# nemochina2008/soundgen_beta

Measured on AMD Instinct MI355X. Metric: synthesized audio samples/sec (whole node) @44.1 kHz; RMS error vs R ref, higher is better.
Workload: dtype fp32 (fp64 phase)

## Files before the change

### include/soundgen_hip.h

```cpp
#ifndef SOUNDGEN_HIP_H
#define SOUNDGEN_HIP_H

#include <stdint.h>

#ifdef __cplusplus
extern "C" {
#endif

#define SG_ABI_VERSION 5

enum {
  SG_OK = 0,
  SG_E_ARG = -1,
  SG_E_DOMAIN = -2,
  SG_E_RANDOM = -3,
  SG_E_UNSUPPORTED = -4,
  SG_E_DEVICE = -5,
  SG_E_CAPACITY = -6,
  SG_E_NOMEM = -7
};

typedef struct sg_anchors {
  int32_t n;
  const double* time;
// ... 114 lines not shown
void sg_plan_destroy(sg_plan* plan);
int64_t sg_plan_n_calls(const sg_plan* plan);
int64_t sg_plan_total_samples(const sg_plan* plan);
int sg_plan_lengths(const sg_plan* plan, int64_t* out_len, int64_t* out_off);
int sg_plan_status(const sg_plan* plan, int32_t* out_status);
int64_t sg_plan_device_bytes(const sg_plan* plan);
int sg_plan_upload(sg_ctx* ctx, sg_plan* plan);
int sg_plan_release_host(sg_plan* plan);
int sg_execute(sg_ctx* ctx, sg_plan* plan, float* d_out, void* stream);
int sg_execute_plans(sg_ctx* ctx, sg_plan* const* plans, float* const* d_outs, int n, void* stream);
int sg_set_profiling(sg_ctx* ctx, int on);
int sg_profile_read(sg_ctx* ctx, double* sine_ms_avg, int64_t* n);
#define SG_PROF_SINE_BANK 0
#define SG_PROF_STFT_OLA 1
int sg_profile_read_kernel(sg_ctx* ctx, int kernel, double* ms_avg, int64_t* n);
int sg_synchronize(sg_ctx* ctx);
int sg_execute_to_host(sg_ctx* ctx, sg_plan* plan, double* out_host);
const char* sg_plan_call_message(const sg_plan* plan, int64_t i);
int sg_plan_kernel_stats(const sg_plan* plan, int64_t* harm_samples,
                         int64_t* harm_terms, int64_t* harm_amp_bytes,
                         int64_t* fft_frames);
int sg_plan_table_stats(const sg_plan* plan, int64_t* tables, int64_t* samples, int64_t* terms);
int sg_plan_stft_stats(const sg_plan* plan, int64_t* samples, int64_t* alg_bytes, double* flops);
int sg_plan_sine_tasks(const sg_plan* plan, int64_t* counts);
int sg_plan_precision(const sg_plan* plan, int32_t* call_fp64, int64_t* fp64_frames, int64_t* fp64_tasks);
int sg_plan_conditioning(const sg_plan* plan, double* rho);
int sg_plan_noise_conditioning(const sg_plan* plan, double* rho);
int sg_plan_call_work(const sg_plan* plan, double* rows, double* fft_flops);
typedef struct sg_mel_params {
  double samplingRate;
  double windowLength;
  double overlap;
  double step;
  double throwaway;
  double maxFreq;
  int32_t penalizeLengthDif;
  int32_t pad;
} sg_mel_params;
int sg_mel_spec(sg_ctx* ctx, const double* wave, int64_t len, const sg_mel_params* p, double* out, int64_t cap,
                int32_t* nb, int32_t* nc);
int sg_compare_sounds_batch(sg_ctx* ctx, const double* target_spec, int32_t nb, int32_t nc_target,
                            const float* d_wave, const int64_t* offsets, const int64_t* lengths, int64_t n,
                            const sg_mel_params* p, int32_t methods, double* out, double* summary);
int sg_dtw_symmetric2(const double* x, int64_t n, const double* y, int64_t m, double* out);
typedef struct sg_ssm_params {
  double samplingRate;
// ... 216 lines not shown
```

### soundgen_beta_amd/batch.py

```python
import ctypes as C

import numpy as np

from . import _abi, native, rargs


class Marshalled:

    def __init__(self, calls):
        self.holder = h = rargs.Holder()
        n = self.n = len(calls)
        N = max(n, 1)
        descs = (_abi.sg_call_desc * N)()
        args = (_abi.sg_soundgen_args * N)()
        self._structs = [args]
        aw = rargs.ArgsWriter(h, args, N)
        fast, rand = [], []
        for i, c in enumerate(calls):
            kind = c.get("kind", "soundgen")
            if kind != "harmonics" and c.get("rng") is None:
                aw.add(i, c.get("args", {}))
                fast.append(i)
                rand.append(h.random_addrs(c.get("normals"), c.get("uniforms")))
                continue
# ... 130 lines not shown
        descs = m.descs
        self._descs = descs
        self.ptr = C.c_void_p()
        L = native.lib()
        native.check(L.sg_plan_batch(ctx.ptr if ctx else None, descs, n, C.byref(self.ptr)), ctx.ptr if ctx else None)
        self.n = n
        self.lengths = np.zeros(n, dtype=np.int64)
        self.offsets = np.zeros(n, dtype=np.int64)
        i64p = C.POINTER(C.c_int64)
        L.sg_plan_lengths(self.ptr, self.lengths.ctypes.data_as(i64p), self.offsets.ctypes.data_as(i64p))
        self.status = np.zeros(n, dtype=np.int32)
        L.sg_plan_status(self.ptr, self.status.ctypes.data_as(C.POINTER(C.c_int32)))
        self.total = int(L.sg_plan_total_samples(self.ptr))
        self.uploaded = False

    def message(self, i):
        return native.lib().sg_plan_call_message(self.ptr, i).decode()

    def stats(self):
        v = [C.c_int64() for _ in range(4)]
        native.lib().sg_plan_kernel_stats(self.ptr, *[C.byref(x) for x in v])
        w = [C.c_int64(), C.c_int64(), C.c_double()]
        native.lib().sg_plan_stft_stats(self.ptr, *[C.byref(x) for x in w])
        return dict(harm_samples=v[0].value, harm_terms=v[1].value, harm_amp_bytes=v[2].value,
                    fft_frames=v[3].value, stft_samples=w[0].value, stft_bytes=w[1].value, stft_flops=w[2].value)

    def sine_tasks(self):
        v = (C.c_int64 * 5)()
        native.check(native.lib().sg_plan_sine_tasks(self.ptr, v))
        return tuple(int(x) for x in v)

    def table_stats(self):
        v = [C.c_int64() for _ in range(3)]
        native.check(native.lib().sg_plan_table_stats(self.ptr, *[C.byref(x) for x in v]))
        return tuple(x.value for x in v)

    def noise_conditioning(self):
        v = np.zeros(self.n, dtype=np.float64)
        native.check(native.lib().sg_plan_noise_conditioning(self.ptr, v.ctypes.data_as(C.POINTER(C.c_double))))
        return v

    def conditioning(self):
        v = np.zeros(self.n, dtype=np.float64)
        native.check(native.lib().sg_plan_conditioning(self.ptr, v.ctypes.data_as(C.POINTER(C.c_double))))
        return v

    def precision(self):
        v = np.zeros(self.n, dtype=np.int32)
# ... 171 lines not shown
```

### soundgen_beta_amd/csrc/sg_api.cpp

```cpp
#include <hip/hip_runtime.h>

#include <algorithm>
#include <cmath>
#include <atomic>
#include <chrono>
#include <cstring>
#include <exception>
#include <memory>
#include <thread>
#include <string>
#include <vector>

#include "sg_plan.h"
#include "sg_exec.h"
#include "sg_amp.h"
#include "sg_prof.h"
#include "sg_mel.h"
#include "sg_launch.h"

#include <cstdio>
#include <cstdlib>

struct sg_plan {
  sg::Batch B;
// ... 654 lines not shown
  *harm_samples = plan->B.harm_samples;
  *harm_terms = plan->B.harm_terms;
  *harm_amp_bytes = plan->B.harm_amp_bytes;
  *fft_frames = plan->B.fft_frames;
  return SG_OK;
}

int sg_plan_table_stats(const sg_plan* plan, int64_t* tables, int64_t* samples, int64_t* terms) {
  if (!plan || !tables || !samples || !terms) return SG_E_ARG;
  *tables = plan->D.uploaded ? (int64_t)plan->D.tabjobs_host.size() : 0;
  *samples = plan->D.uploaded ? plan->D.tab_samples : 0;
  *terms = plan->D.uploaded ? plan->D.tab_terms : 0;
  return SG_OK;
}

int sg_plan_stft_stats(const sg_plan* plan, int64_t* samples, int64_t* alg_bytes, double* flops) {
  if (!plan) return SG_E_ARG;
  *samples = plan->B.stft_samples;
  *alg_bytes = plan->B.stft_bytes;
  *flops = plan->B.stft_flops;
  return SG_OK;
}

int sg_plan_sine_tasks(const sg_plan* plan, int64_t* counts) {
  if (!plan || !counts) return SG_E_ARG;
  const sg::DevicePlan& D = plan->D;
  counts[0] = (int64_t)D.tlong_host.size();
  counts[1] = (int64_t)D.tshort_host.size();
  counts[2] = (int64_t)D.tall_host.size();
  counts[3] = (int64_t)D.tallp_host.size();
  counts[4] = (int64_t)D.thp_host.size();
  return SG_OK;
}

int64_t sg_plan_amp_count(const sg_plan* plan) { return plan && !plan->host_released ? plan->B.amp_total : 0; }

int sg_plan_debug_amps(const sg_plan* plan, float* out, int64_t n) {
  if (!plan || plan->host_released || !out || n < plan->B.amp_total) return SG_E_ARG;
  const sg::Batch& B = plan->B;
  std::vector<double> lg((size_t)B.amp_lg_rows + 1);
  for (size_t k = 0; k < lg.size(); ++k) lg[k] = std::log2((double)(k + 1));
  for (const SgAmpJob& J : B.ampjobs)
    for (int32_t r = 0; r < J.Rp; ++r)
      for (int32_t g = 0; g < J.G; ++g) {
        float a;
        if (r >= J.R) a = 0.f;
// ... 387 lines not shown
```

### soundgen_beta_amd/csrc/sg_dev.h

```cpp
#pragma once
#include <stdint.h>

struct SgSeg {
  double t0;
  double c0, c1, c2, c3, c4;
};

struct SgEpoch {
  int64_t w_off;
  int64_t amp_off;
  int64_t knot_off;
  int32_t seg_off;
  int32_t nseg;
  int32_t n;
  int32_t G;
  int32_t R;
  int32_t u0;
  double x1, xG;
  double xby;
  double invD;
  int32_t dj0, dj1;
  int64_t dk0;
  int32_t syl;
  int32_t pad;
// ... 141 lines not shown

constexpr int SG_FFT_WG = 0;
constexpr int SG_FFT_WAVE = 1;
constexpr int SG_FFT_DFT = 2;
constexpr int SG_FFT_ODD = 3;
constexpr int SG_WAVE_STATE = 24;
constexpr int SG_FFT_WAVES = 8;

#ifndef SG_NOISE_WAVES
#define SG_NOISE_WAVES 12
#endif
constexpr int SG_FFT_WAVES_NOISE = SG_NOISE_WAVES;
constexpr int sg_fft_waves(int phase) { return phase == 0 ? SG_FFT_WAVES_NOISE : SG_FFT_WAVES; }
constexpr int SG_PF_SRC = 20;
constexpr int SG_PF_PAIR = 10;

constexpr int SG_FRAME_FILTER = 0;
constexpr int SG_FRAME_NOISE = 1;
struct SgFrame {
  int64_t src;
  int64_t env;
  int64_t dst;
};
struct SgFrame64 {
  int64_t src;
  int64_t env;
  int64_t dst;
  int32_t wl;
  int32_t mode;
};
constexpr int SG_F64W_M_HOST = 1102;
constexpr int32_t SG_F64_FILTER = 0;
constexpr int32_t SG_F64_NOISE = 1;
struct SgFrameGroup {
  int32_t geom, mode;
  int32_t f0, nf;
};

struct SgOla {
  int64_t frames;
  int64_t out;
  int64_t first, len, xlen;
  double h;
  int32_t nframes, wl;
  float scale;
  int32_t tile0;
// ... 130 lines not shown
```

### soundgen_beta_amd/csrc/sg_fft.hip

```cpp
#include <hip/hip_runtime.h>

#include <type_traits>

#include "sg_dev.h"
#include "sg_devfn.h"
#include "sg_fft64_dev.h"
#include "sg_roots.h"

namespace {

typedef float v2 __attribute__((ext_vector_type(2)));
__device__ __forceinline__ v2 V(float2 a) { return v2{a.x, a.y}; }
__device__ __forceinline__ float2 F(v2 a) { return make_float2(a.x, a.y); }
__device__ __forceinline__ v2 pfma(v2 a, v2 b, v2 c) { return __builtin_elementwise_fma(a, b, c); }
__device__ __forceinline__ v2 splat(float c) { return v2{c, c}; }
__device__ __forceinline__ v2 vmul(v2 a, v2 w) {
  v2 t, r;
  __asm__("v_pk_mul_f32 %0, %1, %2 op_sel_hi:[0,1]" : "=v"(t) : "v"(a), "v"(w));
  __asm__("v_pk_fma_f32 %0, %1, %2, %3 op_sel:[1,1,0] op_sel_hi:[1,0,1] neg_lo:[0,1,0]"
          : "=v"(r) : "v"(a), "v"(w), "v"(t));
  return r;
}
__device__ __forceinline__ v2 vmulc(v2 a, v2 w) {
  v2 t, r;
// ... 885 lines not shown
  auto bstart = [&](int f) -> int { return hi > 0 ? f * hi : (int)floor((double)f * h); };
  const int first = (int)O.first, len = (int)O.len;
  const float scale = O.scale;
  float* out = fs + O.out;
  float m = -INFINITY;
  constexpr bool FUSED = CM == 1102 && R0 == 29 && R1 == 19 && R2 == 2;
  constexpr int CR = FUSED ? 9 : CP;
  float2 C[CR], C2[FUSED ? 9 : 1];
#pragma unroll
  for (int r = 0; r < CR; ++r) C[r] = make_float2(0.f, 0.f);
#pragma unroll
  for (int r = 0; r < (FUSED ? 9 : 1); ++r) C2[r] = make_float2(0.f, 0.f);
  FramePf P;
  constexpr int W = MODE == SG_FRAME_NOISE ? SG_FFT_WAVES_NOISE : SG_FFT_WAVES;
  const float4* A29 = reinterpret_cast<const float4*>(twS + M * (4 + W));
#ifdef SG_STFT_STAMPS
  uint64_t st_accv[10] = {0, 0, 0, 0, 0, 0, 0, 0, 0, 0};
  uint64_t st_lastv = __builtin_amdgcn_s_memtime();
  uint64_t* st_acc = st_accv;
  uint64_t* st_last = &st_lastv;
#endif
  int bf = bstart(S.f0);
  for (int k = 0; k < S.nf; ++k) {
    {
      int Mk = M;
      if (!CM) __asm__ __volatile__("" : "+s"(Mk));
      frame_prefetch<FUSED && MODE == SG_FRAME_FILTER>(P, frames[S.fdev + k], mode, Mk, fl, fs, lane);
    }
    frame_front<CM, R0, R1, R2>(A, P, mode, g, twS, twN, ham, A29, lane SG_ST_ARGS);
    SG_ST(4);
    const float2* han2 = reinterpret_cast<const float2*>(han);
    const bool lastf = k == S.nf - 1;
    const int bn = lastf ? S.pb : bstart(S.f0 + k + 1);
    const int D = bn - bf;
    const bool direct = FUSED && MODE == SG_FRAME_NOISE && bf >= S.pa && bf - first >= 0 && bn - first <= len && D <= 1102;
    if constexpr (FUSED) {
      fft_wc<true, CM, R0, R1, R2, MODE == SG_FRAME_FILTER || SG_NOISE_MFMA, false>(A, twS, A29, lane SG_ST_ARGS);
      float* __restrict__ o = out + (bf - first);
      const bool o2 = ((O.out + bf - first) & 1) == 0;
#pragma unroll
      for (int q = 0; q < 9; ++q) {
        const int j = 64 * q + lane;
        if (j >= 551) continue;
        const float2 a = A[j], c = A[j + 551];
        const float2 t = cmulc(c, twS[550 + j]);
        const float2 y0 = F(pfma(V(cadd(a, t)), V(han2[j]), V(C[q])));
        A[j + 551] = F(pfma(V(csub(a, t)), V(han2[j + 551]), V(C2[q])));
        if (direct && 2 * j < D) {
          const float v0 = y0.x * scale, v1 = y0.y * scale;
          if (2 * j + 1 < D) {
            if (o2) *reinterpret_cast<float2*>(o + 2 * j) = make_float2(v0, v1);
            else {
              o[2 * j] = v0;
              o[2 * j + 1] = v1;
            }
            m = fmaxf(m, fmaxf(v0, v1));
          } else {
            o[2 * j] = v0;
            m = fmaxf(m, v0);
// ... 866 lines not shown
```

### soundgen_beta_amd/csrc/sg_plan.h

```cpp
#pragma once
#include <cstdint>
#include <functional>
#include <memory>
#include <utility>
#include <vector>

#include "sg_dev.h"
#include "sg_rmath.h"
#include "soundgen_hip.h"

namespace sg {

template <class T>
struct NoInitAlloc : std::allocator<T> {
  template <class U>
  struct rebind { using other = NoInitAlloc<U>; };
  NoInitAlloc() = default;
  template <class U>
  NoInitAlloc(const NoInitAlloc<U>&) noexcept {}
  T* allocate(size_t n) {
    if (n * sizeof(T) < SG_BULK_HUGE) return std::allocator<T>::allocate(n);
    return static_cast<T*>(bulk_alloc(n * sizeof(T)));
  }
  void deallocate(T* p, size_t n) noexcept {
// ... 115 lines not shown
  struct UGather {
    const double* src;
    int64_t n, dst, ntot;
  };
  std::vector<UGather> ugath;
  int64_t fu_total = 0, fu_base = 0;
  std::vector<float> ustream;
  std::vector<SgUJob> ujobs;
  std::vector<double> elog2;
  std::vector<int64_t> call_len, call_off;
  std::vector<int32_t> call_status;
  std::vector<int32_t> call_fp64;
  std::vector<double> call_rho;
  double rho_cur = 0;
  std::vector<double> call_rho_noise;
  double rho_noise_cur = 0;
  std::vector<std::string> call_msg;
  int64_t total_out = 0;
  int64_t harm_samples = 0, harm_terms = 0, harm_amp_bytes = 0, fft_frames = 0;
  double fft_flops = 0;
  std::vector<double> call_rows, call_flops;
  int64_t stft_bytes = 0, stft_samples = 0;
  double stft_flops = 0;
};

struct HarmProbe {
  int64_t t;
  double f0;
  std::vector<double> amp;
};
int64_t plan_harmonics(Batch& B, const double* pitch, int64_t len, const sg_harm_params& P,
                       const sg_anchors& amplAnchors, Rng& R, int64_t out_off, bool dry_run, bool to_fs = false,
                       int64_t* fs_off = nullptr, std::vector<HarmProbe>* probes = nullptr);
int64_t syllable_to_fp64(Batch& B, int s);
int64_t fh_alloc(Batch& B, int64_t n);

bool smooth_contour(const sg_anchors& an, int64_t len, bool thisIsPitch, int method, bool has_floor,
                    double vfloor, bool has_ceil, double vceil, vec& out, double sr = 16000);
SgContour contour_desc(Batch& B, const sg_anchors& an, int64_t L, bool has_floor, double vfloor,
                       bool has_ceil, double vceil, bool db, double sr);

void tile_syllables(Batch& B, int first_syl);

int64_t plan_soundgen(Batch& B, const sg_soundgen_args& a, Rng& R, int64_t out_off, int first_syl);
void restore_soundgen_tail(Batch& B, int first_syl);
void finalize_plan(Batch& B);
void finalize_spec(Batch& B);

int geometry(Batch& B, int wl);
int64_t fs_alloc(Batch& B, int64_t n);
int64_t fl_push(Batch& B, const double* v, int64_t n);
int plan_filter(Batch& B, int64_t sound, int64_t L, int wl, double overlap, int64_t env, int64_t env_nc,
                int64_t* out_len, int64_t* out_fs, bool hp = false);
bool plan_noise(Batch& B, Rng& R, int64_t len, const sg_anchors& noiseAnchors, double rolloffNoise,
                double attackLen, int wl, double sr, double overlap, const double* filterNoise, int64_t fnc,
                SgNoiseItem* item, int64_t filt_env = 0);
bool noise_to_fp64(Batch& B, const std::vector<int>& olas);
int64_t plan_envelope(Batch& B, Rng& R, double nrd, int64_t nc, const sg_formants* F, double formantDep,
                      double rolloffLip, const sg_anchors& mouthAnchors, double mouthOpenThres, double openMouthBoost,
                      double vocalTract, double temperature, double formDrift, double formDisp,
                      double formantDepStoch, double smoothLinearFactor, double sr, double speedSound,
                      double slope = 0);
vec sigmoid_half(double sr, double freq, double shape, double spikiness);

vec get_rolloff(const vec& pitch, int64_t nH, const vec& rolloff, const vec& rolloffOct, double rolloffParab,
                double rolloffParabHarm, const vec& rolloffKHz, double baseline, double throwaway, double sr,
                int64_t& H, double rolloffParabCeiling = NAN);
vec get_random_walk(Rng& R, int64_t len, double rw_range, double rw_smoothing, int method, const vec& trend,
                    bool trend_lazy_rnorm, bool draws_only = false);
void clumper(vec& s, const vec& minLen);
double noise_threshold(int which, double nonlinBalance);

}

namespace sg {
int plan_batch_ex(sg_ctx* ctx, const sg_call_desc* calls, int64_t n_calls, bool independent_draws, sg_plan** out,
// ... 5 lines not shown
```

### soundgen_beta_amd/csrc/sg_plan_soundgen.cpp

```cpp
#include <algorithm>
#include <atomic>
#include <cmath>
#include <cstdlib>
#include <cstring>
#include <optional>

#include "sg_plan.h"

namespace sg {

namespace {

constexpr int kNPV = 33;
const char* const kPVNames[kNPV] = {
    "repeatBout", "nSyl", "sylLen", "pauseLen", "temperature", "maleFemale", "creakyBreathy", "nonlinBalance",
    "nonlinDep", "jitterDep", "jitterLen", "vibratoFreq", "vibratoDep", "shimmerDep", "attackLen", "rolloff",
    "rolloffOct", "rolloffParab", "rolloffParabHarm", "rolloffKHz", "rolloffLip", "formantDep", "formantDepStoch",
    "vocalTract", "subFreq", "subDep", "shortestEpoch", "amDep", "amFreq", "amShape", "samplingRate",
    "windowLength", "rolloffNoise"};
const double kPV[kNPV][3] = {
    {1, 1, 20}, {1, 1, 10}, {300, 20, 5000}, {200, 20, 1000}, {.025, 0, 1}, {0, -1, 1}, {0, -1, 1},
    {0, 0, 100}, {50, 0, 100}, {3, 0, 24}, {1, 1, 100}, {5, 3, 10}, {0, 0, 3}, {0, 0, 100},
    {50, 0, 200}, {-12, -60, 0}, {-12, -30, 10}, {0, -50, 50}, {3, 1, 20}, {-6, -20, 0},
    {6, 0, 20}, {1, 0, 5}, {30, 0, 60}, {15.5, 2, 100}, {100, 10, 1000}, {100, 0, 500},
// ... 627 lines not shown
        ci.off = 0;
        B.items.push_back(ci);
        B.mixes[0].push_back(c);
      }
      zero_mix(at, Ls - at);
    } else {
      sound_fs = hp ? fh_alloc(B, std::max<int64_t>(Ls, 1)) : fs_alloc(B, std::max<int64_t>(Ls, 1));
      SgMix pre{};
      pre.dst = sound_fs;
      pre.len = Ls;
      pre.to_fs = hp ? 2 : 1;
      pre.base_kind = SG_BASE_NONE;
      ncontent = emit(sound, pre.item0);
      pre.nitems = ncontent;
      pre.mult = mult;
      B.mixes[0].push_back(pre);
    }
    Layout post;
    if (ncontent == 0) {
      post.items.push_back(raw_item(sound_fs, Ls, 0));
      post.len = Ls;
    } else {
      int64_t filt_fs = 0, Lf = 0;
      const int ola = plan_filter(B, sound_fs, Ls, wl, A.overlap, filt_env, nInt, &Lf, &filt_fs, hp);
      SgNoiseItem fi = raw_item(filt_fs, Lf, 0);
      fi.ola = ola;
      fi.flags = SG_ITEM_FILTER_OLA;
      post.items.push_back(fi);
      post.len = Lf;
    }
    if (postNoise)
      for (size_t s = 0; s < noises.size(); ++s) post.add(noises[s], noiseIp[s]);
    SgMix fin{};
    fin.to_fs = 0;
    fin.base_kind = SG_BASE_NONE;
    fin.len = post.len;
    fin.nitems = emit(post, fin.item0);
    fin.mult.kind = 0;
    if (A.amDep > 0) {
      const vec half = sigmoid_half(sr, A.amFreq, A.amShape, 1);
      fin.am_tab = fl_push(B, half.data(), (int64_t)half.size());
      fin.am_lo = (int32_t)half.size();
      fin.am_dep = (float)A.amDep;
    }
    if (b > 0) {
      const int64_t np = (int64_t)(A.pauseLen * sr / 1000);
      SgMix z{};
// ... 71 lines not shown
```

### soundgen_beta_amd/csrc/sg_plan_spec.cpp

```cpp
#include <algorithm>
#include <atomic>
#include <cmath>
#include <complex>
#include <cstdio>
#include <cstdlib>
#include <cstring>
#include <map>
#include <memory>
#include <mutex>
#include <string>

#include "sg_plan.h"
#include "sg_prof.h"

#ifndef SG_SEG_SORT
#define SG_SEG_SORT 1
#endif
#ifndef SG_ENV_SORT
#define SG_ENV_SORT 1
#endif

namespace sg {

namespace {
// ... 269 lines not shown
}

static int push_ola(Batch& B, int phase, int64_t frames, int64_t nframes, int wl, const IstftGeom& ig, int64_t first,
                    int64_t len, int64_t out, bool fused, bool f64 = false) {
  if (fused && ig.xlen >= (int64_t)1 << 31) throw SgError(SG_E_UNSUPPORTED, "istft: output longer than 2^31 samples");
  SgOla o{};
  o.fidx = f64 ? -1 : (int32_t)((int64_t)B.frames[phase].size() - nframes);
  o.fused = fused ? 1 : 0;
  o.frames = frames;
  o.out = out;
  o.first = first;
  o.len = len;
  o.xlen = ig.xlen;
  o.h = ig.h;
  o.nframes = (int32_t)nframes;
  o.wl = wl;
  o.scale = ig.scale;
  o.hi = (ig.h == std::floor(ig.h) && ig.h >= 1 && ig.h < 2147483647.0) ? (int32_t)ig.h : 0;
  B.olas[phase].push_back(o);
  return (int)B.olas[phase].size() - 1;
}

int plan_filter(Batch& B, int64_t sound, int64_t L, int wl, double overlap, int64_t env, int64_t env_nc,
                int64_t* out_len, int64_t* out_fs, bool hp) {
  ProfScope ps(PF_FILTER);
  const int gi = geometry(B, wl);
  const int64_t nr = wl / 2;
  const double by = (double)wl - overlap * (double)wl / 100;
  const vec step = r_seq_by(1, (double)std::max<int64_t>(1, L - wl), by);
  const int64_t nc = (int64_t)step.size();
  if (env_nc != 1 && env_nc != nc) throw SgError(SG_E_ARG, "formant filter: envelope columns != frames");
  for (double x0 : step)
    if ((int64_t)x0 - 1 + wl > L) throw SgError(SG_E_DOMAIN, "stft: frame beyond the sound");
  const bool fused = !hp && fusable(B.geoms[gi], (double)wl * (100 - overlap) / 100);
  const int64_t fr = fused ? 0 : fs_alloc(B, nc * wl);
  if (hp) {
    for (int64_t c = 0; c < nc; ++c) {
      SgFrame64 f{};
      f.src = sound + (int64_t)step[c] - 1;
      const int64_t col = env_nc == 1 ? 0 : c * nr;
      f.env = env < 0 ? env - col : env + col;
      f.dst = fr + c * wl;
      f.wl = wl;
      B.frames64.push_back(f);
    }
    const IstftGeom ig = istft_geom(wl, nc, overlap);
    const int64_t out = fs_alloc(B, ig.xlen);
    B.fft_frames += nc;
    B.fft_flops += 2 * 5.0 * wl * std::log2((double)wl) * (double)nc;
    *out_len = ig.xlen;
    *out_fs = out;
    return push_ola(B, 1, fr, nc, wl, ig, 0, ig.xlen, out, false, true);
  }
  for (int64_t c = 0; c < nc; ++c) {
    SgFrame f{};
    f.src = sound + (int64_t)step[c] - 1;
    const int64_t col = env_nc == 1 ? 0 : c * nr;
    f.env = env < 0 ? env - col : env + col;
    f.dst = fused ? -1 : fr + c * wl;
    B.frames[1].push_back(f);
    B.frame_geom[1].push_back(gi);
  }
  const IstftGeom ig = istft_geom(wl, nc, overlap);
  const int64_t out = fs_alloc(B, ig.xlen);
  B.fft_frames += nc;
  B.fft_flops += 2 * 5.0 * wl * std::log2((double)wl) * (double)nc;
  *out_len = ig.xlen;
  *out_fs = out;
  return push_ola(B, 1, fr, nc, wl, ig, 0, ig.xlen, out, fused);
}

bool plan_noise(Batch& B, Rng& R, int64_t len, const sg_anchors& noiseAnchors, double rolloffNoise,
                double attackLen, int wl, double sr, double overlap, const double* filterNoise, int64_t fnc,
                SgNoiseItem* item, int64_t filt_env) {
  ProfScope ps(PF_NOISE);
  if (noiseAnchors.n <= 0 || len <= 0) return false;
  SgContour strength = contour_desc(B, noiseAnchors, len, true, -120, true, 40, true, sr);
  const int gi = geometry(B, wl);
  const double hop = (double)wl - overlap * (double)wl / 100;
  const int64_t nc = (int64_t)r_seq_by(1, (double)(len + wl), hop).size();
  const int64_t nr = wl / 2;
  const bool dev = filt_env < 0;
// ... 332 lines not shown
        } else if (rate > 0) {
          const double xhi = 1 + SG_ENV_CUT / L2E / rate * (1 + 1e-6);
          if (std::isfinite(xhi) && xhi < (double)nr - 1) e.khi = (int32_t)std::ceil(xhi) + 1;
        }
        if (!std::isfinite(e.A) || !std::isfinite(e.Rr) || !std::isfinite(e.Lm)) {
          e.klo = 1;
          e.khi = 0;
        }
      }
  }
  if (B.draws_only) return 0;
  job.col0 = (int64_t)B.ecols.size();
  for (int64_t c = 0; c < nc; ++c)
    B.ecols.push_back(SgEnvCol{(float)(rolloffLip * mbin[c]), (float)std::pow(2.0, mouth[c] * openMouthBoost / 10)});
  job.out = B.fe_total;
  B.fe_total += (nr * nc + 63) / 64 * 64;
  B.envjobs.push_back(job);
  return -(job.out + 1);
}

void finalize_spec(Batch& B) {
  B.fe_base = (bulk_size(B.fl_x, B.fl) + 63) / 64 * 64;
  B.fu_base = B.fe_base + (B.fe_total + 63) / 64 * 64;
  for (int ph = 0; ph < 2; ++ph)
    for (SgFrame& f : B.frames[ph]) {
      if (f.env < 0) f.env = B.fe_base + (-f.env - 1);
      if (ph == 0 && f.src < 0) f.src = B.fu_base + (-f.src - 1);
    }
  B.ustream.clear();
  B.ujobs.assign(B.ugath.size(), SgUJob{});
  if (!B.ugath.empty()) {
    std::vector<int64_t> ord(B.ugath.size());
    for (size_t i = 0; i < ord.size(); ++i) ord[i] = (int64_t)i;
    auto lo = [&](int64_t i) { return (uintptr_t)B.ugath[i].src; };
    std::sort(ord.begin(), ord.end(), [&](int64_t a, int64_t b) { return lo(a) < lo(b); });
    size_t k = 0;
    while (k < ord.size()) {
      const double* r0 = B.ugath[ord[k]].src;
      uintptr_t end = lo(ord[k]) + 8 * (uintptr_t)B.ugath[ord[k]].n;
      size_t k1 = k + 1;
      while (k1 < ord.size() && lo(ord[k1]) <= end) {
        end = std::max<uintptr_t>(end, lo(ord[k1]) + 8 * (uintptr_t)B.ugath[ord[k1]].n);
        ++k1;
      }
      const int64_t base = (int64_t)B.ustream.size(), n = (int64_t)((end - (uintptr_t)r0) / 8);
      B.ustream.resize((size_t)(base + n));
      for (int64_t j = 0; j < n; ++j) B.ustream[(size_t)(base + j)] = (float)r0[j];
      for (size_t q = k; q < k1; ++q) {
// ... 20 lines not shown
    B.frames64_w[1] = std::stable_partition(mid, B.frames64.end(), w) - mid;
  }
  for (SgFrame64& f : B.frames64) {
    if (f.env < 0) f.env = B.fe_base + (-f.env - 1);
    if (f.mode == SG_F64_NOISE && f.src < 0) f.src = B.fu_base + (-f.src - 1);
    size_t w = 0;
    while (w < B.roots64_wl.size() && B.roots64_wl[w] != f.wl) ++w;
    if (w == B.roots64_wl.size()) {
      B.roots64_wl.push_back(f.wl);
      B.roots64_off.push_back(B.roots64_total);
      B.roots64_total += 2 * (int64_t)f.wl;
    }
    B.frames64_tab.push_back(B.roots64_off[w]);
    B.frames64_maxwl = std::max(B.frames64_maxwl, f.wl);
  }
  int32_t maxnr = 0;
  for (const SgEnvJob& j : B.envjobs) {
    maxnr = std::max(maxnr, j.nr);
    if (j.ntr > 2 * 64) throw SgError(SG_E_DEVICE, "spectral envelope: more than 128 formant tracks (planner check)");
  }
  B.elog2.resize((size_t)std::max<int64_t>(maxnr, B.amp_lg_rows) + 64);
  for (size_t k = 0; k < B.elog2.size(); ++k) B.elog2[k] = std::log2((double)(k + 1));
  B.envtasks.clear();
  for (size_t j = 0; j < B.envjobs.size(); ++j)
    for (int32_t c0 = 0; c0 < B.envjobs[j].nc; c0 += SG_ENV_COLS) B.envtasks.push_back(SgEnvTask{(int32_t)j, c0});
  auto cost = [&](const SgEnvTask& t) {
    const SgEnvJob& J = B.envjobs[t.job];
    return (double)std::min<int32_t>(SG_ENV_COLS, J.nc - t.c0) * (double)((J.nr + 127) / 128) * (double)J.ntr;
  };
  if (SG_ENV_SORT)
    std::stable_sort(B.envtasks.begin(), B.envtasks.end(),
                     [&](const SgEnvTask& a, const SgEnvTask& b) { return cost(a) > cost(b); });
  if (std::getenv("SG_DEBUG_PLAN")) {
    double wmax = 0, wsum = 0;
    for (size_t i = 0; i < B.envtasks.size(); i += 4) {
      double mx = 0;
      for (size_t w = i; w < i + 4 && w < B.envtasks.size(); ++w) { mx = std::max(mx, cost(B.envtasks[w])); wsum += cost(B.envtasks[w]); }
      wmax += 4 * mx;
    }
    std::fprintf(stderr, "sg plan: envelope tasks %zu, workgroup cost %.3g, used %.3g (%.1f%% idle)\n", B.envtasks.size(), wmax,
                 wsum, wmax > 0 ? 100.0 * (wmax - wsum) / wmax : 0.0);
  }
  B.fgroups.clear();
  std::vector<int64_t> pos[2];
  for (int ph = 0; ph < 2; ++ph) {
    const size_t ng = B.geoms.size();
    std::vector<int64_t> rank(ng), start(ng + 1, 0);
    {
// ... 42 lines not shown
  B.olas_dev.clear();
  B.olatiles.clear();
  B.olasegs.clear();
  B.ola_split = (int64_t)B.olas[0].size();
  for (int ph = 0; ph < 2; ++ph) {
    if (ph == 1) B.olatile_split = (int64_t)B.olatiles.size();
    const int32_t base = ph == 0 ? 0 : (int32_t)B.frames[0].size();
    for (const SgOla& o0 : B.olas[ph]) {
      SgOla o = o0;
      if (o0.fidx >= 0) o.fidx = base + (int32_t)pos[ph][o0.fidx];
      const int32_t oi = (int32_t)B.olas_dev.size();
      if (!o.fused) {
        o.tile0 = (int32_t)B.olatiles.size();
        for (int64_t q0 = 0; q0 < o.len; q0 += SG_OLA_TILE) B.olatiles.push_back(SgOlaTile{oi, 0, q0});
        o.nslot = (int32_t)B.olatiles.size() - o.tile0;
      }
      B.olas_dev.push_back(o);
    }
  }
  const int32_t nt = (int32_t)B.olatiles.size();
  int32_t nslots = 0;
  B.stft_bytes = B.stft_samples = 0;
  B.stft_flops = 0;
  for (int ph = 0; ph < 2; ++ph) {
    B.seg_range[ph][0] = (int64_t)B.olasegs.size();
    const size_t o_lo = ph == 0 ? 0 : (size_t)B.ola_split, o_hi = ph == 0 ? (size_t)B.ola_split : B.olas_dev.size();
    const int32_t fbase = ph == 0 ? 0 : (int32_t)B.frames[0].size();
    const int WPH = sg_fft_waves(ph);
    std::vector<size_t> order;
    for (size_t oi = o_lo; oi < o_hi; ++oi)
      if (B.olas_dev[oi].fused) order.push_back(oi);
    auto geom_of = [&](size_t oi) { return B.frame_geom[ph][B.olas_dev[oi].fidx - fbase]; };
    std::stable_sort(order.begin(), order.end(), [&](size_t a, size_t b) { return geom_of(a) < geom_of(b); });
    const int64_t SEG = sg_seg_frames(ph);
    int64_t seg_frames = SEG;
    {
      auto segs_at = [&](int64_t S) {
        int64_t tot = 0, run = 0;
        int prev = -2;
        for (size_t oi : order) {
          const int g = geom_of(oi);
          if (g != prev) {
            tot += (WPH - run % WPH) % WPH;
            run = 0;
            prev = g;
          }
          const int64_t k = std::max<int64_t>(1, (B.olas_dev[oi].nframes + S - 1) / S);
          tot += k;
          run += k;
        }
        return tot + (WPH - run % WPH) % WPH;
      };
      const int64_t base = segs_at(SEG);
      const int64_t rounds = (base + sg_resident_waves(ph) - 1) / sg_resident_waves(ph);
      int64_t S = SG_SEG_MIN_FRAMES;
      while (S < SEG && segs_at(S) > rounds * sg_resident_waves(ph)) S = std::max(S + 1, S * 9 / 8);
      seg_frames = std::min<int64_t>(S, SEG);
    }
    int cur_geom = -1;
    size_t group0 = B.olasegs.size();
    auto pad = [&]() {
      if (SG_SEG_SORT)
        std::stable_sort(B.olasegs.begin() + (std::ptrdiff_t)group0, B.olasegs.end(),
                         [](const SgSegment& a, const SgSegment& b) { return a.nf > b.nf; });
      while (((int64_t)B.olasegs.size() - B.seg_range[ph][0]) % WPH) {
        SgSegment d{};
        d.geom = cur_geom;
        B.olasegs.push_back(d);
      }
    };
    for (size_t oi : order) {
      SgOla& o = B.olas_dev[oi];
      const int gi = geom_of(oi);
      if (gi != cur_geom) {
        pad();
        cur_geom = gi;
        group0 = B.olasegs.size();
      }
      auto bstart = [&](int64_t f) -> int64_t {
        return o.hi > 0 ? f * o.hi : (int64_t)std::floor((double)f * o.h);
      };
      const int64_t n = o.nframes;
      const int64_t nseg = std::max<int64_t>(1, (n + seg_frames - 1) / seg_frames);
      {
        const int64_t nr = o.wl / 2;
        int64_t ncol = 0, prev = -1;
        for (int64_t f = 0; f < n; ++f) {
          const int64_t e = B.frames[ph][o.fidx - fbase + f].env;
          if (e != prev) ++ncol;
          prev = e;
        }
        const double fft = 5.0 * o.wl * std::log2((double)o.wl);
        if (ph == 0) {
          B.stft_bytes += 4 * (nr * n + nr * ncol + o.len);
          B.stft_flops += fft * n;
        } else {
          B.stft_bytes += 4 * (std::min<int64_t>(o.xlen, o.wl + (int64_t)std::ceil((n - 1) * o.h)) + nr * ncol + o.len);
          B.stft_flops += 2 * fft * n;
        }
        B.stft_samples += o.len;
      }
      o.tile0 = nt + nslots;
      o.nslot = (int32_t)nseg;
      for (int64_t k = 0; k < nseg; ++k) {
        const int64_t F0 = k * n / nseg, F1 = (k + 1) * n / nseg;
        SgSegment sg{};
        sg.ola = (int32_t)oi;
        sg.geom = gi;
        sg.mode = ph == 0 ? SG_FRAME_NOISE : SG_FRAME_FILTER;
        sg.pa = k == 0 ? 0 : (int32_t)bstart(F0);
        sg.pb = k == nseg - 1 ? (int32_t)o.xlen : (int32_t)bstart(F1);
        int64_t f0 = F0;
        while (f0 > 0 && bstart(f0 - 1) + o.wl > sg.pa) --f0;
        sg.f0 = (int32_t)f0;
        sg.nf = (int32_t)(F1 - f0);
        sg.fdev = o.fidx + (int32_t)f0;
        sg.slot = nt + nslots++;
        sg.flags = (k == 0 ? SG_SEG_FIRST : 0) | (k == nseg - 1 ? SG_SEG_LAST : 0);
        B.olasegs.push_back(sg);
      }
    }
    pad();
    B.seg_range[ph][1] = (int64_t)B.olasegs.size();
  }
  B.n_segslots = nslots;
  if (std::getenv("SG_DEBUG_PLAN")) {
    int64_t owned = 0, run = 0, real = 0;
    for (const SgSegment& sg : B.olasegs) {
      if (sg.nf <= 0) continue;
      ++real;
      run += sg.nf;
    }
    for (const SgOla& o : B.olas_dev) if (o.fused) owned += o.nframes;
    for (int ph = 0; ph < 2; ++ph) {
      int64_t fr = 0, sgs = 0;
      for (int64_t i = B.seg_range[ph][0]; i < B.seg_range[ph][1]; ++i)
        if (B.olasegs[i].nf > 0) { fr += B.olasegs[i].nf; ++sgs; }
      std::fprintf(stderr, "sg plan: phase %d: %lld frames computed in %lld segments (%zu frames, %zu unfused groups)\n", ph,
                   (long long)fr, (long long)sgs, B.frames[ph].size(), (size_t)(B.fgroup_range[ph][2] - B.fgroup_range[ph][1]));
      const int WPH = sg_fft_waves(ph);
      int64_t wmax = 0, wsum = 0;
      for (int64_t i = B.seg_range[ph][0]; i < B.seg_range[ph][1]; i += WPH) {
        int64_t mx = 0;
        for (int w = 0; w < WPH && i + w < B.seg_range[ph][1]; ++w) mx = std::max<int64_t>(mx, B.olasegs[i + w].nf);
        wmax += mx * WPH;
        for (int w = 0; w < WPH && i + w < B.seg_range[ph][1]; ++w) wsum += std::max<int32_t>(0, B.olasegs[i + w].nf);
      }
      std::fprintf(stderr, "sg plan: phase %d: workgroup wave-frames %lld, used %lld (%.1f%% idle)\n", ph, (long long)wmax,
                   (long long)wsum, wmax ? 100.0 * (double)(wmax - wsum) / (double)wmax : 0.0);
    }
    std::map<int32_t, int64_t> gfr;
    for (const SgSegment& sg : B.olasegs)
      if (sg.nf > 0) gfr[sg.geom] += sg.nf;
    std::vector<std::pair<int64_t, int32_t>> gs;
    for (const auto& kv : gfr) gs.push_back({kv.second, kv.first});
    std::sort(gs.rbegin(), gs.rend());
    for (size_t i = 0; i < gs.size() && i < 16; ++i) {
      const SgFftGeom& g = B.geoms[gs[i].second];
      std::string rs;
      for (int s = 0; s < g.nstages; ++s) rs += (s ? "x" : "") + std::to_string(g.radix[s]);
      std::fprintf(stderr, "sg plan: geom wl=%d M=%d radices %s: %lld frames\n", g.wl, g.M, rs.c_str(),
                   (long long)gs[i].first);
    }
    std::map<int32_t, int64_t> gun;
    for (const SgFrameGroup& fg : B.fgroups) gun[fg.geom] += fg.nf;
    for (const auto& kv : gun) {
      const SgFftGeom& g = B.geoms[kv.first];
      std::string rs;
      for (int s = 0; s < g.nstages; ++s) rs += (s ? "x" : "") + std::to_string(g.radix[s]);
      std::fprintf(stderr, "sg plan: unfused geom wl=%d M=%d kind %d radices %s: %lld frames\n", g.wl, g.M, g.kind,
                   rs.c_str(), (long long)kv.second);
    }
// ... 34 lines not shown
```

### soundgen_beta_amd/native.py

```python
import ctypes as C
import os
import re

from . import _abi

_HERE = os.path.dirname(os.path.abspath(__file__))
LIB_PATH = os.environ.get("SG_HIP_LIB") or os.path.join(_HERE, "lib", "libsoundgen_hip.so")
HEADER_PATH = os.path.join(os.path.dirname(_HERE), "include", "soundgen_hip.h")

_lib = None
HP_RHO_DEFAULT = 100.0


class SoundgenError(RuntimeError):
    def __init__(self, code, msg):
        super().__init__("%s: %s" % (_abi.SG_ERR_NAMES.get(code, code), msg))
        self.code = code


def declared_symbols():
    txt = open(HEADER_PATH).read()
    txt = re.sub(r"/\*.*?\*/", "", txt, flags=re.S)
    return sorted(set(re.findall(r"\b(sg_[a-z_0-9]+)\s*\(", txt)))

# ... 17 lines not shown
    L.sg_ctx_destroy.argtypes = [vp]
    L.sg_last_error.argtypes = [vp]
    L.sg_last_error.restype = C.c_char_p
    L.sg_plan_batch.argtypes = [vp, C.POINTER(_abi.sg_call_desc), i64, C.POINTER(vp)]
    L.sg_plan_destroy.argtypes = [vp]
    L.sg_plan_n_calls.argtypes = [vp]
    L.sg_plan_n_calls.restype = i64
    L.sg_plan_total_samples.argtypes = [vp]
    L.sg_plan_total_samples.restype = i64
    L.sg_plan_lengths.argtypes = [vp, i64p, i64p]
    L.sg_plan_status.argtypes = [vp, C.POINTER(C.c_int32)]
    L.sg_plan_call_message.argtypes = [vp, i64]
    L.sg_plan_call_message.restype = C.c_char_p
    L.sg_plan_device_bytes.argtypes = [vp]
    L.sg_plan_device_bytes.restype = i64
    L.sg_plan_upload.argtypes = [vp, vp]
    L.sg_plan_release_host.argtypes = [vp]
    L.sg_execute.argtypes = [vp, vp, vp, vp]
    L.sg_execute_plans.argtypes = [vp, C.POINTER(vp), C.POINTER(vp), C.c_int, vp]
    L.sg_set_profiling.argtypes = [vp, C.c_int]
    L.sg_profile_read.argtypes = [vp, dp, i64p]
    L.sg_profile_read_kernel.argtypes = [vp, C.c_int, dp, i64p]
    L.sg_plan_stft_stats.argtypes = [vp, i64p, i64p, dp]
    L.sg_plan_conditioning.argtypes = [vp, dp]
    L.sg_plan_noise_conditioning.argtypes = [vp, dp]
    L.sg_plan_precision.argtypes = [vp, C.POINTER(C.c_int32), i64p, i64p]
    L.sg_set_fp64_policy.argtypes = [C.c_int32, C.c_double]
    L.sg_set_amp_policy.argtypes = [C.c_int32]
    L.sg_set_uniform_gather.argtypes = [C.c_int32]
    if hasattr(L, "sg_plan_sine_tasks"):
        L.sg_plan_sine_tasks.argtypes = [vp, i64p]
    L.sg_set_sine_table.argtypes = [C.c_int32]
    L.sg_plan_table_stats.argtypes = [C.c_void_p, C.POINTER(i64), C.POINTER(i64), C.POINTER(i64)]
    L.sg_host_cache_trim.argtypes = []
    L.sg_host_cache_trim.restype = i64
    L.sg_get_smooth_contour.argtypes = [_abi.sg_anchors, C.c_int64, C.c_int32, C.c_int32, C.c_int32, C.c_double,
                                        C.c_int32, C.c_double, C.c_double, C.POINTER(C.c_double),
                                        C.POINTER(C.c_int64)]
    L.sg_plan_amp_count.restype = C.c_int64
    L.sg_plan_amp_count.argtypes = [C.c_void_p]
    L.sg_plan_debug_amps.argtypes = [C.c_void_p, C.POINTER(C.c_float), C.c_int64]
    L.sg_plan_call_work.argtypes = [vp, dp, dp]
    L.sg_dtw_symmetric2.argtypes = [dp, i64, dp, i64, dp]
    L.sg_mel_spec.argtypes = [vp, dp, i64, C.POINTER(_abi.sg_mel_params), dp, i64, C.POINTER(C.c_int32),
                              C.POINTER(C.c_int32)]
    L.sg_compare_sounds_batch.argtypes = [vp, dp, C.c_int32, C.c_int32, vp, i64p, i64p, i64,
# ... 224 lines not shown
```

Before: 14.07 billion.

## Skip FFT filtering of all-zero STFT frames and their envelope columns

At plan time, filter frames whose window overlaps no nonzero sound item are marked zero. The kernel then skips the prefetch, forward FFT and filter for those frames and writes a constant or zero spectrum. Envelope columns read only by such frames are left out of the envelope task list. Segments are sorted by a cost that counts zero frames as cheap, to balance waves. The change adds an env-var toggle, a stats API and plan-time scanning cost, and it relies on the zero-frame output being exactly equivalent to the real one.

```diff
diff --git a/include/soundgen_hip.h b/include/soundgen_hip.h
--- a/include/soundgen_hip.h
+++ b/include/soundgen_hip.h
@@ -160,6 +160,7 @@
                          int64_t* fft_frames);
 int sg_plan_table_stats(const sg_plan* plan, int64_t* tables, int64_t* samples, int64_t* terms);
 int sg_plan_stft_stats(const sg_plan* plan, int64_t* samples, int64_t* alg_bytes, double* flops);
+int64_t sg_plan_zero_frames(const sg_plan* plan);
 int sg_plan_sine_tasks(const sg_plan* plan, int64_t* counts);
 int sg_plan_precision(const sg_plan* plan, int32_t* call_fp64, int64_t* fp64_frames, int64_t* fp64_tasks);
 int sg_plan_conditioning(const sg_plan* plan, double* rho);
diff --git a/soundgen_beta_amd/batch.py b/soundgen_beta_amd/batch.py
--- a/soundgen_beta_amd/batch.py
+++ b/soundgen_beta_amd/batch.py
@@ -176,8 +176,11 @@
         native.lib().sg_plan_kernel_stats(self.ptr, *[C.byref(x) for x in v])
         w = [C.c_int64(), C.c_int64(), C.c_double()]
         native.lib().sg_plan_stft_stats(self.ptr, *[C.byref(x) for x in w])
+        L = native.lib()
+        zero = int(L.sg_plan_zero_frames(self.ptr)) if hasattr(L, "sg_plan_zero_frames") else 0
         return dict(harm_samples=v[0].value, harm_terms=v[1].value, harm_amp_bytes=v[2].value,
-                    fft_frames=v[3].value, stft_samples=w[0].value, stft_bytes=w[1].value, stft_flops=w[2].value)
+                    fft_frames=v[3].value, stft_samples=w[0].value, stft_bytes=w[1].value, stft_flops=w[2].value,
+                    stft_zero_frames=zero)
 
     def sine_tasks(self):
         v = (C.c_int64 * 5)()
diff --git a/soundgen_beta_amd/csrc/sg_api.cpp b/soundgen_beta_amd/csrc/sg_api.cpp
--- a/soundgen_beta_amd/csrc/sg_api.cpp
+++ b/soundgen_beta_amd/csrc/sg_api.cpp
@@ -700,6 +700,8 @@
   return SG_OK;
 }
 
+int64_t sg_plan_zero_frames(const sg_plan* plan) { return plan ? plan->B.stft_zero_frames : 0; }
+
 int sg_plan_sine_tasks(const sg_plan* plan, int64_t* counts) {
   if (!plan || !counts) return SG_E_ARG;
   const sg::DevicePlan& D = plan->D;
diff --git a/soundgen_beta_amd/csrc/sg_dev.h b/soundgen_beta_amd/csrc/sg_dev.h
--- a/soundgen_beta_amd/csrc/sg_dev.h
+++ b/soundgen_beta_amd/csrc/sg_dev.h
@@ -187,6 +187,8 @@
   int64_t env;
   int64_t dst;
 };
+constexpr int64_t SG_FRAME_ZERO = -2;
+constexpr int64_t SG_FRAME_ZERO_OWN = -3;
 struct SgFrame64 {
   int64_t src;
   int64_t env;
diff --git a/soundgen_beta_amd/csrc/sg_fft.hip b/soundgen_beta_amd/csrc/sg_fft.hip
--- a/soundgen_beta_amd/csrc/sg_fft.hip
+++ b/soundgen_beta_amd/csrc/sg_fft.hip
@@ -931,19 +931,39 @@
 #endif
   int bf = bstart(S.f0);
   for (int k = 0; k < S.nf; ++k) {
-    {
+    const bool zf = MODE == SG_FRAME_FILTER && frames[S.fdev + k].env < 0;
+    if (!zf) {
       int Mk = M;
       if (!CM) __asm__ __volatile__("" : "+s"(Mk));
       frame_prefetch<FUSED && MODE == SG_FRAME_FILTER>(P, frames[S.fdev + k], mode, Mk, fl, fs, lane);
-    }
-    frame_front<CM, R0, R1, R2>(A, P, mode, g, twS, twN, ham, A29, lane SG_ST_ARGS);
+      frame_front<CM, R0, R1, R2>(A, P, mode, g, twS, twN, ham, A29, lane SG_ST_ARGS);
+    }
     SG_ST(4);
     const float2* han2 = reinterpret_cast<const float2*>(han);
     const bool lastf = k == S.nf - 1;
     const int bn = lastf ? S.pb : bstart(S.f0 + k + 1);
     const int D = bn - bf;
     const bool direct = FUSED && MODE == SG_FRAME_NOISE && bf >= S.pa && bf - first >= 0 && bn - first <= len && D <= 1102;
-    if constexpr (FUSED) {
+    if (zf) {
+      if constexpr (FUSED) {
+#pragma unroll
+        for (int q = 0; q < 9; ++q) {
+          const int j = 64 * q + lane;
+          if (j >= 551) continue;
+          A[j] = C[q];
+          A[j + 551] = C2[q];
+        }
+      } else {
+        int Mk = M;
+        if (!CM) __asm__ __volatile__("" : "+s"(Mk));
+#pragma unroll
+        for (int r = 0; r < CP; ++r) {
+          const int n = 64 * r + lane;
+          if (n < Mk) A[n] = C[r];
+        }
+        for (int n = 64 * CP + lane; n < Mk; n += 64) A[n] = make_float2(0.f, 0.f);
+      }
+    } else if constexpr (FUSED) {
       fft_wc<true, CM, R0, R1, R2, MODE == SG_FRAME_FILTER || SG_NOISE_MFMA, false>(A, twS, A29, lane SG_ST_ARGS);
       float* __restrict__ o = out + (bf - first);
       const bool o2 = ((O.out + bf - first) & 1) == 0;
diff --git a/soundgen_beta_amd/csrc/sg_plan.h b/soundgen_beta_amd/csrc/sg_plan.h
--- a/soundgen_beta_amd/csrc/sg_plan.h
+++ b/soundgen_beta_amd/csrc/sg_plan.h
@@ -161,6 +161,7 @@
   std::vector<double> call_rows, call_flops;
   int64_t stft_bytes = 0, stft_samples = 0;
   double stft_flops = 0;
+  int64_t stft_zero_frames = 0;
 };
 
 struct HarmProbe {
@@ -190,7 +191,8 @@
 int64_t fs_alloc(Batch& B, int64_t n);
 int64_t fl_push(Batch& B, const double* v, int64_t n);
 int plan_filter(Batch& B, int64_t sound, int64_t L, int wl, double overlap, int64_t env, int64_t env_nc,
-                int64_t* out_len, int64_t* out_fs, bool hp = false);
+                int64_t* out_len, int64_t* out_fs, bool hp = false,
+                const std::vector<std::pair<int64_t, int64_t>>* content = nullptr);
 bool plan_noise(Batch& B, Rng& R, int64_t len, const sg_anchors& noiseAnchors, double rolloffNoise,
                 double attackLen, int wl, double sr, double overlap, const double* filterNoise, int64_t fnc,
                 SgNoiseItem* item, int64_t filt_env = 0);
diff --git a/soundgen_beta_amd/csrc/sg_plan_soundgen.cpp b/soundgen_beta_amd/csrc/sg_plan_soundgen.cpp
--- a/soundgen_beta_amd/csrc/sg_plan_soundgen.cpp
+++ b/soundgen_beta_amd/csrc/sg_plan_soundgen.cpp
@@ -673,7 +673,10 @@
       post.len = Ls;
     } else {
       int64_t filt_fs = 0, Lf = 0;
-      const int ola = plan_filter(B, sound_fs, Ls, wl, A.overlap, filt_env, nInt, &Lf, &filt_fs, hp);
+      std::vector<std::pair<int64_t, int64_t>> content;
+      for (const auto& it : sound.items)
+        if (!(it.flags & SG_ITEM_ZERO) && it.len > 0) content.push_back({it.off, it.off + it.len});
+      const int ola = plan_filter(B, sound_fs, Ls, wl, A.overlap, filt_env, nInt, &Lf, &filt_fs, hp, &content);
       SgNoiseItem fi = raw_item(filt_fs, Lf, 0);
       fi.ola = ola;
       fi.flags = SG_ITEM_FILTER_OLA;
diff --git a/soundgen_beta_amd/csrc/sg_plan_spec.cpp b/soundgen_beta_amd/csrc/sg_plan_spec.cpp
--- a/soundgen_beta_amd/csrc/sg_plan_spec.cpp
+++ b/soundgen_beta_amd/csrc/sg_plan_spec.cpp
@@ -315,7 +315,7 @@
 }
 
 int plan_filter(Batch& B, int64_t sound, int64_t L, int wl, double overlap, int64_t env, int64_t env_nc,
-                int64_t* out_len, int64_t* out_fs, bool hp) {
+                int64_t* out_len, int64_t* out_fs, bool hp, const std::vector<std::pair<int64_t, int64_t>>* content) {
   ProfScope ps(PF_FILTER);
   const int gi = geometry(B, wl);
   const int64_t nr = wl / 2;
@@ -345,12 +345,21 @@
     *out_fs = out;
     return push_ola(B, 1, fr, nc, wl, ig, 0, ig.xlen, out, false, true);
   }
+  const char* zenv = std::getenv("SG_ZERO_FRAMES");
+  const bool skip_zero = !(zenv && zenv[0] == '0');
   for (int64_t c = 0; c < nc; ++c) {
     SgFrame f{};
     f.src = sound + (int64_t)step[c] - 1;
     const int64_t col = env_nc == 1 ? 0 : c * nr;
     f.env = env < 0 ? env - col : env + col;
     f.dst = fused ? -1 : fr + c * wl;
+    if (fused && content && skip_zero) {
+      const int64_t a = (int64_t)step[c] - 1, b = a + wl;
+      bool zero = true;
+      for (const auto& sp : *content)
+        if (sp.first < b && sp.second > a) { zero = false; break; }
+      if (zero) f.dst = env < 0 && env_nc == nc && nc > 1 ? SG_FRAME_ZERO_OWN : SG_FRAME_ZERO;
+    }
     B.frames[1].push_back(f);
     B.frame_geom[1].push_back(gi);
   }
@@ -729,8 +738,25 @@
 void finalize_spec(Batch& B) {
   B.fe_base = (bulk_size(B.fl_x, B.fl) + 63) / 64 * 64;
   B.fu_base = B.fe_base + (B.fe_total + 63) / 64 * 64;
+  std::vector<uint8_t> col_unread(B.ecols.size(), 0);
+  B.stft_zero_frames = 0;
   for (int ph = 0; ph < 2; ++ph)
     for (SgFrame& f : B.frames[ph]) {
+      if (ph == 1 && f.dst <= SG_FRAME_ZERO) {
+        if (f.dst == SG_FRAME_ZERO_OWN && f.env < 0) {
+          const int64_t off = -f.env - 1;
+          auto it = std::upper_bound(B.envjobs.begin(), B.envjobs.end(), off,
+                                     [](int64_t o, const SgEnvJob& j) { return o < j.out; });
+          if (it != B.envjobs.begin()) {
+            const SgEnvJob& J = *(it - 1);
+            const int64_t c = (off - J.out) / J.nr;
+            if (c < J.nc && (off - J.out) % J.nr == 0) col_unread[(size_t)(J.col0 + c)] = 1;
+          }
+        }
+        f.env = -1;
+        ++B.stft_zero_frames;
+        continue;
+      }
       if (f.env < 0) f.env = B.fe_base + (-f.env - 1);
       if (ph == 0 && f.src < 0) f.src = B.fu_base + (-f.src - 1);
     }
@@ -797,8 +823,17 @@
   B.elog2.resize((size_t)std::max<int64_t>(maxnr, B.amp_lg_rows) + 64);
   for (size_t k = 0; k < B.elog2.size(); ++k) B.elog2[k] = std::log2((double)(k + 1));
   B.envtasks.clear();
-  for (size_t j = 0; j < B.envjobs.size(); ++j)
-    for (int32_t c0 = 0; c0 < B.envjobs[j].nc; c0 += SG_ENV_COLS) B.envtasks.push_back(SgEnvTask{(int32_t)j, c0});
+  for (size_t j = 0; j < B.envjobs.size(); ++j) {
+    const SgEnvJob& J = B.envjobs[j];
+    for (int32_t c0 = 0; c0 < J.nc;) {
+      if (col_unread[(size_t)(J.col0 + c0)]) {
+        ++c0;
+        continue;
+      }
+      B.envtasks.push_back(SgEnvTask{(int32_t)j, c0});
+      c0 += SG_ENV_COLS;
+    }
+  }
   auto cost = [&](const SgEnvTask& t) {
     const SgEnvJob& J = B.envjobs[t.job];
     return (double)std::min<int32_t>(SG_ENV_COLS, J.nc - t.c0) * (double)((J.nr + 127) / 128) * (double)J.ntr;
@@ -887,6 +922,13 @@
   int32_t nslots = 0;
   B.stft_bytes = B.stft_samples = 0;
   B.stft_flops = 0;
+  auto seg_cost = [&](const SgSegment& sg) -> int64_t {
+    if (sg.mode != SG_FRAME_FILTER || B.stft_zero_frames == 0) return 8 * (int64_t)std::max<int32_t>(0, sg.nf);
+    const SgFrame* f = B.frames[1].data() + (sg.fdev - (int64_t)B.frames[0].size());
+    int64_t c = 0;
+    for (int32_t k = 0; k < sg.nf; ++k) c += f[k].env < 0 ? 1 : 8;
+    return c;
+  };
   for (int ph = 0; ph < 2; ++ph) {
     B.seg_range[ph][0] = (int64_t)B.olasegs.size();
     const size_t o_lo = ph == 0 ? 0 : (size_t)B.ola_split, o_hi = ph == 0 ? (size_t)B.ola_split : B.olas_dev.size();
@@ -925,9 +967,13 @@
     int cur_geom = -1;
     size_t group0 = B.olasegs.size();
     auto pad = [&]() {
-      if (SG_SEG_SORT)
-        std::stable_sort(B.olasegs.begin() + (std::ptrdiff_t)group0, B.olasegs.end(),
-                         [](const SgSegment& a, const SgSegment& b) { return a.nf > b.nf; });
+      if (SG_SEG_SORT) {
+        std::vector<std::pair<int64_t, SgSegment>> v;
+        v.reserve(B.olasegs.size() - group0);
+        for (size_t i = group0; i < B.olasegs.size(); ++i) v.push_back({seg_cost(B.olasegs[i]), B.olasegs[i]});
+        std::stable_sort(v.begin(), v.end(), [](const auto& a, const auto& b) { return a.first > b.first; });
+        for (size_t i = 0; i < v.size(); ++i) B.olasegs[group0 + i] = v[i].second;
+      }
       while (((int64_t)B.olasegs.size() - B.seg_range[ph][0]) % WPH) {
         SgSegment d{};
         d.geom = cur_geom;
@@ -952,6 +998,7 @@
         int64_t ncol = 0, prev = -1;
         for (int64_t f = 0; f < n; ++f) {
           const int64_t e = B.frames[ph][o.fidx - fbase + f].env;
+          if (e < 0) continue;
           if (e != prev) ++ncol;
           prev = e;
         }
@@ -990,6 +1037,8 @@
   }
   B.n_segslots = nslots;
   if (std::getenv("SG_DEBUG_PLAN")) {
+    std::fprintf(stderr, "sg plan: %lld zero filter frames of %zu (%.2f%%)\n", (long long)B.stft_zero_frames,
+                 B.frames[1].size(), B.frames[1].empty() ? 0.0 : 100.0 * (double)B.stft_zero_frames / (double)B.frames[1].size());
     int64_t owned = 0, run = 0, real = 0;
     for (const SgSegment& sg : B.olasegs) {
       if (sg.nf <= 0) continue;
@@ -1007,12 +1056,12 @@
       int64_t wmax = 0, wsum = 0;
       for (int64_t i = B.seg_range[ph][0]; i < B.seg_range[ph][1]; i += WPH) {
         int64_t mx = 0;
-        for (int w = 0; w < WPH && i + w < B.seg_range[ph][1]; ++w) mx = std::max<int64_t>(mx, B.olasegs[i + w].nf);
+        for (int w = 0; w < WPH && i + w < B.seg_range[ph][1]; ++w) mx = std::max<int64_t>(mx, seg_cost(B.olasegs[i + w]));
         wmax += mx * WPH;
-        for (int w = 0; w < WPH && i + w < B.seg_range[ph][1]; ++w) wsum += std::max<int32_t>(0, B.olasegs[i + w].nf);
-      }
-      std::fprintf(stderr, "sg plan: phase %d: workgroup wave-frames %lld, used %lld (%.1f%% idle)\n", ph, (long long)wmax,
-                   (long long)wsum, wmax ? 100.0 * (double)(wmax - wsum) / (double)wmax : 0.0);
+        for (int w = 0; w < WPH && i + w < B.seg_range[ph][1]; ++w) wsum += seg_cost(B.olasegs[i + w]);
+      }
+      std::fprintf(stderr, "sg plan: phase %d: workgroup wave-frames %lld, used %lld (%.1f%% idle)\n", ph, (long long)(wmax / 8),
+                   (long long)(wsum / 8), wmax ? 100.0 * (double)(wmax - wsum) / (double)wmax : 0.0);
     }
     std::map<int32_t, int64_t> gfr;
     for (const SgSegment& sg : B.olasegs)
diff --git a/soundgen_beta_amd/native.py b/soundgen_beta_amd/native.py
--- a/soundgen_beta_amd/native.py
+++ b/soundgen_beta_amd/native.py
@@ -63,6 +63,9 @@
     L.sg_profile_read.argtypes = [vp, dp, i64p]
     L.sg_profile_read_kernel.argtypes = [vp, C.c_int, dp, i64p]
     L.sg_plan_stft_stats.argtypes = [vp, i64p, i64p, dp]
+    if hasattr(L, "sg_plan_zero_frames"):
+        L.sg_plan_zero_frames.argtypes = [vp]
+        L.sg_plan_zero_frames.restype = i64
     L.sg_plan_conditioning.argtypes = [vp, dp]
     L.sg_plan_noise_conditioning.argtypes = [vp, dp]
     L.sg_plan_precision.argtypes = [vp, C.POINTER(C.c_int32), i64p, i64p]
```

Measured after the change: 14.05 billion. About the same (-0.1%).
